# stephane-caron/pink

Hardware: AMD Instinct MI355X
Metric: ik_qp_solves_per_s (higher is better)
Workload: dtype f64

## Files before the change

__graft_entry__.py:

```python

from __future__ import annotations

import hashlib
import os
import subprocess
import sys

ROOT = os.path.dirname(os.path.abspath(__file__))
CSRC = os.path.join(ROOT, "pink_amd", "csrc")
LIB = os.path.join(CSRC, "libpinkhip.so")
HIP_DEPS = ["Makefile", "pinkhip.hip", "tu_kernel.hip", "object_list.h", "ik_sweep.h", "ik_sweepx.h", "ik_stack_rows.h", "ik_rollout.h", "ik_common.h", "ik_kernels_packed.h", "ik_stack_mfma.h",
            "ik_frame_task.h", "ik_kinematics.h", "model_tables.h", "wave.h", "fast_sincos.h", "host_tables.h", "host_plan.h", "dispatch.h",
            "launchers.h", os.path.join(ROOT, "include", "pinkhip.h")]
STAMP = os.path.join(CSRC, "libpinkhip.srchash")


def _source_hash(deps) -> str:
    h = hashlib.sha256()
    for d in deps:
        p = d if os.path.isabs(d) else os.path.join(CSRC, d)
        h.update(os.path.basename(p).encode() + b"\0")
        with open(p, "rb") as f:
            h.update(f.read())
    return h.hexdigest()


def _fresh(target: str, stamp: str, want: str) -> bool:
    return os.path.exists(target) and os.path.exists(stamp) and open(stamp).read().strip() == want


class _BuildLock:

    def __init__(self, name: str):
        self.path = os.path.join(CSRC, name)

    def __enter__(self):
        import fcntl

        self.f = open(self.path, "w")
        fcntl.flock(self.f, fcntl.LOCK_EX)
        return self

    def __exit__(self, *exc):
        import fcntl

        fcntl.flock(self.f, fcntl.LOCK_UN)
        self.f.close()


def build_hip(force: bool = False) -> str:
    want = _source_hash(HIP_DEPS)
    if force or not _fresh(LIB, STAMP, want):
        with _BuildLock(".build.lock"):
            if force or not _fresh(LIB, STAMP, want):
                jobs = str(max(1, len(os.sched_getaffinity(0))))
                subprocess.check_call(["make", "-j", jobs], cwd=CSRC)
                with open(STAMP, "w") as f:
                    f.write(want + "\n")
    return LIB


EMU_PARTS = 16


def build_emulator(force: bool = False) -> str:
    from concurrent.futures import ThreadPoolExecutor

    emu_dir = os.path.join(ROOT, "emu")
    out_dir = os.path.join(ROOT, "tests", "emu")
    target = os.path.join(out_dir, "libpinkemu.so")
    harness = sorted(f for f in os.listdir(emu_dir) if f.startswith("emu_") and f.endswith(".cpp") and not f.endswith("_part.cpp"))
    deps = [os.path.join(emu_dir, f) for f in harness + ["emu_part.cpp", "emu_lanes.h", "emu_registry.h", "wave_emu.h"]] + [WAVE_PROBE_KERNEL, MASK_PROBE_KERNEL] + \
           [os.path.join(CSRC, f) for f in ("ik_common.h", "dispatch.h", "wave.h", "fast_sincos.h", "ik_kernels_packed.h", "ik_sweep.h", "ik_sweepx.h", "ik_stack_rows.h",
                                            "ik_rollout.h", "ik_stack_mfma.h", "ik_frame_task.h", "ik_kinematics.h", "model_tables.h", "host_tables.h", "host_plan.h")]
    stamp, want = os.path.join(out_dir, "libpinkemu.srchash"), _source_hash(deps)
    if force or not _fresh(target, stamp, want):
        with _BuildLock(".build_emu.lock"):
            if force or not _fresh(target, stamp, want):
                objdir = os.path.join(emu_dir, "build")
                os.makedirs(objdir, exist_ok=True)
                os.makedirs(out_dir, exist_ok=True)
                cxx = ["g++", "-O1", "-std=c++17", "-fPIC", "-Wno-psabi"]
                jobs = [cxx + ["-c", os.path.join(emu_dir, f), "-o", os.path.join(objdir, f[:-4] + ".o")] for f in harness]
                for k in range(EMU_PARTS):
                    jobs.append(cxx + [f"-DEMU_PART={k}", f"-DEMU_NPARTS={EMU_PARTS}", "-c", os.path.join(emu_dir, "emu_part.cpp"),
                                       "-o", os.path.join(objdir, f"emu_part_{k}.o")])
                workers = max(1, min(len(jobs), len(os.sched_getaffinity(0))))
                with ThreadPoolExecutor(workers) as pool:
                    list(pool.map(subprocess.check_call, jobs))
                objs = [j[-1] for j in jobs]
                subprocess.check_call(["g++", "-shared", "-o", target + ".tmp"] + objs)
                os.replace(target + ".tmp", target)
                with open(stamp, "w") as f:
                    f.write(want + "\n")
    return target


WAVE_PROBE_DIR = os.path.join(ROOT, "tests", "wave")
WAVE_PROBE_KERNEL = os.path.join(WAVE_PROBE_DIR, "wave_probe_kernel.h")
WAVE_PROBE_LIB = os.path.join(WAVE_PROBE_DIR, "libwaveprobe.so")
MASK_PROBE_KERNEL = os.path.join(WAVE_PROBE_DIR, "lane_mask_probe_kernel.h")
MASK_PROBE_LIB = os.path.join(WAVE_PROBE_DIR, "liblanemaskprobe.so")


def _build_probe(source: str, kernel: str, lib: str, force: bool) -> str:
    deps = [os.path.join(WAVE_PROBE_DIR, source), kernel, os.path.join(CSRC, "wave.h"), os.path.join(CSRC, "fast_sincos.h")]
    stamp, want = lib[:-3] + ".srchash", _source_hash(deps)
    if force or not _fresh(lib, stamp, want):
        with _BuildLock(".build_probe.lock"):
            if force or not _fresh(lib, stamp, want):
                import shutil

                hipcc = os.environ.get("HIPCC") or shutil.which("hipcc") or "/opt/rocm/bin/hipcc"
                subprocess.check_call([hipcc, "--offload-arch=gfx950", "-O3", "-std=c++17", "-fPIC", "-shared", deps[0], "-o", lib + ".tmp"])
                os.replace(lib + ".tmp", lib)
                with open(stamp, "w") as f:
                    f.write(want + "\n")
    return lib


def build_wave_probe(force: bool = False) -> str:
    return _build_probe("wave_probe.hip", WAVE_PROBE_KERNEL, WAVE_PROBE_LIB, force)


def build_lane_mask_probe(force: bool = False) -> str:
    return _build_probe("lane_mask_probe.hip", MASK_PROBE_KERNEL, MASK_PROBE_LIB, force)


def build() -> None:
    build_hip()
    build_wave_probe()
    build_lane_mask_probe()
    sys.path.insert(0, ROOT)
    from oracle import c_oracle

    c_oracle.build()
    build_emulator()
    import pink_amd
    from pink_amd import _lib

    lib = _lib.load_library()
    for name in _lib.ABI_SYMBOLS:
        getattr(lib, name)


def smoke() -> None:
    sys.path.insert(0, ROOT)
    import numpy as np

    from oracle import c_oracle
    from pink_amd import synthetic
    from pink_amd.batch_solver import BatchSolver

    build_hip()
    solver = BatchSolver(device_id=0)
    try:
        for name, B in (("ur5", 64), ("draco3", 256), ("jvrc", 64)):
            terms = synthetic.make_terms(name, B, bounds="tight")
            ref = c_oracle.solve_ik_batch(**synthetic.pink_form(terms))
            out = solver.solve(synthetic.pack(terms))
            assert (out.status == 0).all() and (ref["status"] == 0).all()
            err = float(np.abs(out.dq - ref["dq"]).max())
            print(f"smoke {name}: B={B} max|dq - dq_ref| = {err:.3e}")
            assert err < 1e-8, err
    finally:
        solver.close()


if __name__ == "__main__":
    build()
    if len(sys.argv) > 1 and sys.argv[1] == "smoke":
        smoke()
```

pink_amd/csrc/ik_common.h:

```cpp
#pragma once

#include <cmath>
#include <cstdint>
#include <type_traits>

#ifndef PINKHIP_GROUP_LARGE
#define PINKHIP_GROUP_LARGE 8
#endif
#ifndef PINKHIP_GROUP_SMALL
#define PINKHIP_GROUP_SMALL 4
#endif

#if defined(PINKHIP_TRACE) && !defined(__HIP_DEVICE_COMPILE__)
#include <cstdio>
#define PINKHIP_TRACEF(cond, ...)        \
  do {                                   \
    if (cond) std::printf(__VA_ARGS__);  \
  } while (0)
#else
#define PINKHIP_TRACEF(cond, ...)
#endif

namespace pinkhip {

template <int NV>
constexpr int group_size() {
  return NV >= 24 ? PINKHIP_GROUP_LARGE : PINKHIP_GROUP_SMALL;
}

template <int I, int N, class F>
__device__ __forceinline__ void static_for(F &&f) {
  if constexpr (I < N) {
    f(std::integral_constant<int, I>{});
    static_for<I + 1, N>(f);
  }
}
template <int W, int J>
__device__ __forceinline__ double add_in_lane(double t, double d) {
  static_assert((W == 16 || W == 32 || W == 64) && J >= 0 && J < W, "lane of a group of whole rows of 16 lanes");
#if defined(__HIP_DEVICE_COMPILE__)
  constexpr unsigned long long one = 1ull << J;
  constexpr unsigned long long m = W == 64 ? one : W == 32 ? one | (one << 32) : one | (one << 16) | (one << 32) | (one << 48);
  unsigned slo, shi;
  asm("s_mov_b32 %1, exec_lo\n\ts_mov_b32 %2, exec_hi\n\t"
      "s_and_b32 exec_lo, %1, %4\n\ts_and_b32 exec_hi, %2, %5\n\t"
      "v_add_f64 %0, %0, %3\n\t"
      "s_mov_b32 exec_lo, %1\n\ts_mov_b32 exec_hi, %2"
      : "+v"(t), "=&s"(slo), "=&s"(shi)
      : "v"(d), "n"(static_cast<int>(m & 0xFFFFFFFFull)), "n"(static_cast<int>(m >> 32))
      : "scc");
  return t;
#else
  return ((lane_id() & (W - 1)) == J) ? t + d : t;
#endif
}

template <int W, int N, int BIT, class F>
__device__ __forceinline__ double transpose_reduce(F v) {
  const int lane = lane_id();
  if constexpr ((1 << BIT) >= W) {
    static_assert(N == 1, "N <= W values fold to one per lane");
    return v(std::integral_constant<int, 0>{});
  } else {
    constexpr int H = (N + 1) / 2;
    double nx[H];
    const bool up = ((lane >> BIT) & 1) != 0;
    static_for<0, H>([&](auto M) {
      constexpr int m = decltype(M)::value;
      const double a = v(std::integral_constant<int, 2 * m>{});
      double b = 0.0;
      if constexpr (2 * m + 1 < N) b = v(std::integral_constant<int, 2 * m + 1>{});
      nx[m] = (up ? b : a) + lane_shfl(up ? a : b, lane ^ (1 << BIT));
    });
    return transpose_reduce<W, H, BIT + 1>([&](auto K) { return nx[decltype(K)::value]; });
  }
}

typedef double TabVec16 __attribute__((vector_size(128)));
typedef double TabVec8 __attribute__((vector_size(64)));
template <bool HALF>
struct TabVecSel {
  typedef TabVec16 type;
};
template <>
struct TabVecSel<true> {
  typedef TabVec8 type;
};
template <int NT>
struct TabRegs {
  static constexpr int NVEC = (NT + 15) / 16;
  static_assert(NVEC >= 1 && NVEC <= 4, "at most 64 tableau columns");
  static constexpr bool kHalfLast = NT - 16 * (NVEC - 1) <= 8;
  template <int K>
  using Vec = typename TabVecSel<(K == NVEC - 1) && kHalfLast>::type;
  Vec<0> v0;
  Vec<1> v1;
  Vec<2> v2;
  Vec<3> v3;
  template <int K>
  __device__ __forceinline__ Vec<K> tuple() const {
    if constexpr (K == 0) return v0;
    else if constexpr (K == 1) return v1;
    else if constexpr (K == 2) return v2;
    else return v3;
  }
  template <int J>
  __device__ __forceinline__ double get() const {
    static_assert(J >= 0 && J < NT, "tableau column");
    const Vec<J / 16> t = tuple<J / 16>();
    return t[J % 16];
  }
  template <int J>
  __device__ __forceinline__ void set(double x) {
    static_assert(J >= 0 && J < NT, "tableau column");
    Vec<J / 16> t = tuple<J / 16>();
    t[J % 16] = x;
    if constexpr (J / 16 == 0) v0 = t;
    else if constexpr (J / 16 == 1) v1 = t;
    else if constexpr (J / 16 == 2) v2 = t;
    else v3 = t;
  }
  __device__ __forceinline__ void clear() {
    v0 = Vec<0>{};
    v1 = Vec<1>{};
    v2 = Vec<2>{};
    v3 = Vec<3>{};
  }
  __device__ __forceinline__ double at_uniform(int p) const {
    const int hi = p >> 4;
    const int lo = opaque_uniform(p & 15);
    const int lo8 = kHalfLast ? opaque_uniform(p & 7) : lo;
    const Vec<0> t0 = v0;
    double r = t0[NVEC == 1 ? lo8 : lo];
    if constexpr (NVEC > 1) {
      const Vec<1> t1 = v1;
      const double r1 = t1[NVEC == 2 ? lo8 : lo];
      r = (hi == 1) ? r1 : r;
    }
    if constexpr (NVEC > 2) {
      const Vec<2> t2 = v2;
      const double r2 = t2[NVEC == 3 ? lo8 : lo];
      r = (hi == 2) ? r2 : r;
    }
    if constexpr (NVEC > 3) {
      const Vec<3> t3 = v3;
      const double r3 = t3[lo8];
      r = (hi == 3) ? r3 : r;
    }
    return r;
  }
  template <int W>
  __device__ __forceinline__ double at_group_uniform(int p) const {
    constexpr int G = kWave / W;
    static_assert(G == 1 || G == 2, "one or two reads per wave");
    const int p0 = bcast_i(p, 0);
    double c = at_uniform(p0 < 0 ? 0 : p0);
    if constexpr (G == 2) {
      const int p1 = bcast_i(p, W);
      const double c1 = at_uniform(p1 < 0 ? 0 : p1);
      c = (lane_id() >= W) ? c1 : c;
    }
    return (p >= 0) ? c : 0.0;
  }
};

struct alignas(16) Pair {
  double a, b;
};

constexpr int STATUS_OPTIMAL = 0;
constexpr int STATUS_MAX_ITER = 1;
constexpr int STATUS_INFEASIBLE = 2;
constexpr int STATUS_NOT_PD = 3;
constexpr int STATUS_BREAKDOWN = 4;
constexpr int STATUS_ROUTED = 5;
constexpr int PATH_TABLEAU = 0, PATH_HANDOVER = 1, PATH_ROUTED = 2, PATH_GI = 3;
constexpr int kPathShift = 24;

struct KernelArgs {
  long long B;
  int nv, Kd, K, md;
  int n_eq;
  int n_dtasks;
  int n_barriers;
  int cost_batched;
  int max_iter;
  int lds_pitch;
  int rank_deficient;
  int n_free_lead;
  double damping, dt;
  double out_scale;
  const double *J, *e, *cost, *lb, *ub, *Gd, *hd, *c_extra;
  const double *row_gain;
  const double *row_lm;
  const int *dtask_col0;
  const int *dtask_row0;
  const int *dtask_k;
  const int *barrier_rows;
  const double *barrier_safe_gain;
  double *dq;
  int *status;
  int *iters;
  double *H_out, *c_out;
  const uint8_t *active_in;
  uint8_t *active_out;
};


}
```

pink_amd/csrc/ik_sweep.h:

```cpp
#pragma once

#include "ik_common.h"
#include "ik_kernels_packed.h"
#include "ik_stack_rows.h"

#ifdef PINKHIP_SECTION_CLOCK
#ifndef PINKHIP_TICK
static __device__ unsigned long long pinkhip_clock[16];
#define PINKHIP_TICK(k)                                                        \
  do {                                                                         \
    if (clock_on) {                                                            \
      const unsigned long long now_ = __builtin_readcyclecounter();            \
      if (lane == 0) atomicAdd(&pinkhip_clock[k], now_ - clock_prev);          \
      clock_prev = __builtin_readcyclecounter();                               \
    }                                                                          \
  } while (0)
#endif
#else
#ifndef PINKHIP_TICK
#define PINKHIP_TICK(k)
#endif
#endif

#ifndef PINKHIP_SWEEP_COLUMN_CHAINS
#define PINKHIP_SWEEP_COLUMN_CHAINS(NT) 2
#endif

#ifndef PINKHIP_SWEEP_CERT_TOL
#define PINKHIP_SWEEP_CERT_TOL 1e-12
#endif
#ifndef PINKHIP_STACK_DEPTH
#define PINKHIP_STACK_DEPTH 1
#endif
#ifndef PINKHIP_STACK_DEPTH_WIDE
#define PINKHIP_STACK_DEPTH_WIDE 2
#endif
#ifndef PINKHIP_SWEEP_INDEXED_COLUMN
#define PINKHIP_SWEEP_INDEXED_COLUMN 1
#endif
#ifndef PINKHIP_SWEEP_ROUTE_COND
#define PINKHIP_SWEEP_ROUTE_COND 1e8
#endif
#ifndef PINKHIP_SWEEP_PPM
#define PINKHIP_SWEEP_PPM 1
#endif
#ifndef PINKHIP_SWEEP_PPM_CRASH
#define PINKHIP_SWEEP_PPM_CRASH 1
#endif
#ifndef PINKHIP_ROLLOUT_PPM_DENSE
#define PINKHIP_ROLLOUT_PPM_DENSE 0
#endif
#ifndef PINKHIP_ROLLOUT_PPM_VIRTUAL
#define PINKHIP_ROLLOUT_PPM_VIRTUAL 0
#endif
#ifndef PINKHIP_SWEEP_PPM_DENSE
#define PINKHIP_SWEEP_PPM_DENSE 1
#endif
#ifdef PINKHIP_SWEEP_DEBUG_WHY
#define PINKHIP_WHY(k) why = (k) + 10 * status_before
#else
#define PINKHIP_WHY(k)
#endif
#ifndef PINKHIP_SWEEP_PPM_MIN_CURV
#define PINKHIP_SWEEP_PPM_MIN_CURV 1e-5
#endif
#ifndef PINKHIP_SWEEP_PPM_MURTY_AFTER
#define PINKHIP_SWEEP_PPM_MURTY_AFTER(nv) (4 * (nv) + 20)
#endif

#ifndef PINKHIP_SWEEP_DIAG_REGISTER
#define PINKHIP_SWEEP_DIAG_REGISTER(Src) (!Src::kOnTheFly)
#endif
#ifndef PINKHIP_SWEEP_LATE_ADDRESSES
#define PINKHIP_SWEEP_LATE_ADDRESSES(Src) (!Src::kOnTheFly)
#endif
#ifndef PINKHIP_SWEEP_LANE_MASKS
#define PINKHIP_SWEEP_LANE_MASKS(Src) (!Src::kOnTheFly)
#endif

namespace pinkhip {

template <int NV, int MD, int W>
struct SweepLds {
  static __host__ __device__ constexpr int tri(int i) { return i * (i + 1) / 2; }
  static constexpr int oC = (NV * (NV + 1) / 2 + 1) & ~1;
  static constexpr int GP = W + 2;
  static constexpr int oG = oC + W;
  static constexpr int oR = oG + MD * GP;
  static constexpr int stride = oR + W;
};

template <int NVT, int MD, int W, class Src = HbmTerms, bool WARM = false>
__device__ __forceinline__ int ik_sweep_instance(const KernelArgs &a, long long block, Src *terms = nullptr) {
  constexpr int NE = NVT > W ? NVT - W : 0;
  constexpr int NV = NVT - NE;
  static_assert(NE == 0 || (NE <= 2 && MD == 0 && !Src::kOnTheFly), "front coordinates are eliminated in the box-only stack + solve kernel");
  constexpr int NT = NV + MD;
  static_assert((W == 16 || W == 32 || W == 64) && NT <= W && NV % 2 == 0 && MD >= 0, "group of whole rows of 16 lanes");
  constexpr bool DENSE = MD > 0;
  constexpr bool DREG = PINKHIP_SWEEP_DIAG_REGISTER(Src);
  constexpr bool LM = PINKHIP_SWEEP_LANE_MASKS(Src);
  constexpr bool PPM = !DENSE && PINKHIP_SWEEP_PPM;
  constexpr bool PPMD = DENSE && PINKHIP_SWEEP_PPM && PINKHIP_SWEEP_PPM_DENSE && (!Src::kOnTheFly || PINKHIP_ROLLOUT_PPM_DENSE);
  constexpr bool PPX = PPM || PPMD;
  constexpr bool LMP = LM && PPM;
  static_assert(!WARM || PPM, "a warm start is a start of the principal pivoting of the box-only instantiations");
  constexpr int G = kWave / W;
  constexpr double INF = INFINITY;
  constexpr double BIG = 1e300;
  using BcT = Bcast<W>;

  const int lane = lane_id();
  const int g = lane / W, li = lane & (W - 1);
  const int nvs = a.nv;
  const int nv = nvs - NE;
  const int md = DENSE ? a.md : 0, n_eq = DENSE ? a.n_eq : 0;
#ifdef PINKHIP_SECTION_CLOCK
  const bool clock_on = (block & 63) == 0;
  unsigned long long clock_prev = __builtin_readcyclecounter();
#endif
  long long b = block * G + g;
  const bool valid = b < a.B;
  if (!valid) b = a.B - 1;
  WaveSplit ws;
  ws.first = (block * G < a.B - 1) ? block * G : a.B - 1;
  ws.rel = static_cast<unsigned>(b - ws.first);
  const unsigned vo = ws.rel * static_cast<unsigned>(nvs) + li;

  const bool in = li < nv;
  const int dr = li - NV;
  const bool dlane = DENSE && dr >= 0 && dr < md;

  double T[NT];
#pragma unroll
  for (int j = 0; j < NT; ++j) T[j] = 0.0;
  double ci = 0.0, mu_l = 0.0, dadd = 0.0;
  double ci_d = 0.0, mu_d = 0.0, lbv = -INF, ubv = INF, hv = 0.0, ginv = 1.0;
  double front_dadd[NE > 0 ? NE : 1] = {}, front_c[NE > 0 ? NE : 1] = {};
  bool front_free = true;
  auto others = [&]() {
    if (in) {
      if constexpr (!Src::kOnTheFly) {
        lbv = (a.lb + (ws.first * (long long)nvs + NE))[vo];
        ubv = (a.ub + (ws.first * (long long)nvs + NE))[vo];
      }
      if constexpr (PINKHIP_WAVE_SPLIT(Src)) dadd = stack_diag_tasks<Src>(a, ws, terms, NE + li, ci_d, mu_d);
      else dadd = stack_diag_tasks<Src>(a, b, terms, NE + li, ci_d, mu_d);
      if constexpr (PINKHIP_WAVE_SPLIT(Src)) {
        if (a.c_extra) ci_d += (a.c_extra + (ws.first * (long long)nvs + NE))[vo];
      } else {
        if (a.c_extra) ci_d += a.c_extra[b * (long long)nvs + NE + li];
      }
    }
    if constexpr (NE > 0) {
#pragma unroll
      for (int x = 0; x < NE; ++x) {
        double mu_x = 0.0;
        front_dadd[x] = stack_diag_tasks<Src>(a, b, terms, x, front_c[x], mu_x);
        if (a.c_extra) front_c[x] += a.c_extra[b * (long long)nvs + x];
        if (li == x) mu_d += mu_x;
        front_free = front_free && a.lb[b * (long long)nvs + x] == -INF && a.ub[b * (long long)nvs + x] == INF;
      }
    }
    if constexpr (DENSE && !Src::kOnTheFly) {
      if (md > 0) {
        const double *Gb = a.Gd + b * (long long)md * nv;
        static_for<0, MD>([&](auto Dc) {
          constexpr int d = decltype(Dc)::value;
          T[NV + d] = (in && d < md) ? Gb[(long long)d * nv + li] : 0.0;
        });
        if (dlane) hv = a.hd[b * (long long)md + dr];
      }
    }
  };
  StackFront<NE> front;
  double hii = 0.0;
  if constexpr (NE > 0) {
    KernelArgs af = a;
    af.J = a.J + NE;
    stack_rows_bcast<NV, W, 8, Src, PINKHIP_STACK_DEPTH, NE, DREG>(af, b, terms, in, li, T, ci, mu_l, others, &front, &hii, ws);
  } else {
    stack_rows_bcast<NV, W, 8, Src, (NT > 34 ? PINKHIP_STACK_DEPTH_WIDE : PINKHIP_STACK_DEPTH), 0, DREG>(a, b, terms, in, li, T, ci, mu_l, others, nullptr, &hii, ws);
  }
  ci += ci_d;
  mu_l += mu_d;
  double diag = a.damping + group_sum<W>(mu_l);

  if constexpr (DENSE) {
    if (md > 0) {
      const double *Gb = Src::kOnTheFly ? nullptr : a.Gd + b * (long long)md * nv;
      if constexpr (Src::kOnTheFly) {
        static_for<0, MD>([&](auto Dc) {
          constexpr int d = decltype(Dc)::value;
          T[NV + d] = (in && d < md) ? terms->dense_col(d) : 0.0;
        });
      }
      if constexpr (Src::kOnTheFly) {
        static_for<0, MD>([&](auto Dc) {
          constexpr int d = decltype(Dc)::value;
          if (d < md) {
            const BcT gb = bcast_prepare<W>(T[NV + d]);
            static_for<0, NV>([&](auto Jc) {
              constexpr int j = decltype(Jc)::value;
              const double v = value_bcast<W, j>(gb);
              if (dr == d) T[j] = v;
            });
          }
        });
      }
      if (dlane) {
        double n2 = 0.0;
        if constexpr (!Src::kOnTheFly) {
          const double *gr = Gb + (long long)dr * nv;
#pragma unroll
          for (int j = 0; j < NV; ++j) T[j] = (j < nv) ? gr[j] : 0.0;
        } else {
          hv = terms->dense_h(dr);
        }
#pragma unroll
        for (int j = 0; j < NV; ++j) n2 += T[j] * T[j];
        ginv = (n2 > 0.0) ? 1.0 / sqrt(n2) : 1.0;
      }
      for (int t = 0; t < a.n_barriers; ++t) {
        const double r = a.barrier_safe_gain[t];
        if (r > 1e-6) {
          const int r0 = a.barrier_rows[t], r1 = a.barrier_rows[t + 1];
          double s = 0.0;
          static_for<0, MD>([&](auto Dc) {
            constexpr int d = decltype(Dc)::value;
            if (in && d >= r0 && d < r1) s += T[NV + d] * T[NV + d];
          });
          s = group_sum<W>(s);
          diag += r / (s * a.dt * a.dt);
        }
      }
    }
  }
  const double diag_u = diag;
  diag += dadd;
  if constexpr (DREG) {
    const double dd = in ? diag : 1.0;
    static_for<0, NV>([&](auto Jc) {
      constexpr int j = decltype(Jc)::value;
      T[j] = add_in_lane<W, j>(T[j], dd);
    });
    hii += dd;
  } else {
    hii = 1.0;
#pragma unroll
    for (int j = 0; j < NV; ++j)
      if (j == li) {
        T[j] += in ? diag : 1.0;
        hii = T[j];
      }
  }
  using SL = SweepLds<NV, MD, W>;
  double *sm = shared_base() + (long long)g * (a.lds_pitch ? a.lds_pitch : SL::stride);
  bool front_bad = false;
  if constexpr (NE > 0) {
    double h00 = group_sum<W>(front.hxx[0]) + diag_u + front_dadd[0];
    double c0 = group_sum<W>(front.cx[0]) + front_c[0];
    double h01 = 0.0, h11 = 1.0, c1 = 0.0;
    if constexpr (NE == 2) {
      h01 = group_sum<W>(front.hxx[1]);
      h11 = group_sum<W>(front.hxx[2]) + diag_u + front_dadd[1];
      c1 = group_sum<W>(front.cx[1]) + front_c[1];
    }
    const double m0 = in ? front.m[0] : 0.0;
    double m1 = (NE == 2 && in) ? front.m[NE - 1] : 0.0;
    front_bad = !(h00 > 0.0);
    const double r0 = fast_rcp(h00);
    {
      const BcT hb = bcast_prepare<W>(m0);
      const double f = -m0 * r0;
      static_for<0, NV>([&](auto Jc) {
        constexpr int j = decltype(Jc)::value;
        T[j] = fma_bcast<W, j>(T[j], hb, f);
      });
      ci = fma(f, c0, ci);
      hii = fma(f, m0, hii);
      if constexpr (NE == 2) {
        m1 = fma(f, h01, m1);
        h11 = fma(-h01 * r0, h01, h11);
        c1 = fma(-h01 * r0, c0, c1);
      }
    }
    double r1 = 0.0;
    if constexpr (NE == 2) {
      front_bad = front_bad || !(h11 > 0.0);
      r1 = fast_rcp(h11);
      const BcT hb = bcast_prepare<W>(m1);
      const double f = -m1 * r1;
      static_for<0, NV>([&](auto Jc) {
        constexpr int j = decltype(Jc)::value;
        T[j] = fma_bcast<W, j>(T[j], hb, f);
      });
      ci = fma(f, c1, ci);
      hii = fma(f, m1, hii);
    }
    wave_sync();
    sm[SL::stride + li] = m0;
    sm[SL::stride + W + li] = m1;
    if (li == 0) {
      double *fs = sm + SL::stride + 2 * W;
      fs[0] = c0, fs[1] = r0, fs[2] = h01, fs[3] = c1, fs[4] = r1;
    }
  }
  wave_sync();
  if (li < NV) {
#pragma unroll
    for (int j = 0; j < NV; ++j)
      if (j <= li) sm[SL::tri(li) + j] = T[j];
  }
  sm[SL::oC + li] = ci;
  if constexpr (DENSE) {
    static_for<0, MD>([&](auto Dc) {
      constexpr int d = decltype(Dc)::value;
      sm[SL::oG + d * SL::GP + li] = (li < NV) ? T[NV + d] : 0.0;
    });
  }
  PINKHIP_TICK(0);

  int status = STATUS_OPTIMAL;
  int why = 0, status_before = 0;
  if constexpr (NE > 0) {
    if (!front_free) status = STATUS_ROUTED;
    else if (front_bad) status = STATUS_NOT_PD;
  }
  double pmin = INF;
  int state = 0;
  if constexpr (Src::kOnTheFly) {
    lbv = in ? terms->lb : -INF;
    ubv = in ? terms->ub : INF;
  }
  constexpr bool GUESS = (PPX && PINKHIP_SWEEP_PPM_CRASH && !Src::kOnTheFly) || WARM;
  double tdiag = (li < NV) ? hii : 0.0;
  if constexpr (GUESS) {
    if (group_first_lane<W>(in && !(hii > 0.0)) < W) status = STATUS_NOT_PD;
    if constexpr (WARM) {
      const uint8_t *hint = a.active_in;
      if (hint) {
        if (in) {
          const int v = hint[b * (long long)nvs + NE + li];
          state = (v == 1 && lbv > -INF) ? 1 : ((v == 2 && ubv < INF) ? 2 : 0);
        }
      } else if constexpr (!Src::kOnTheFly) {
        const double xd = -ci * approx_rcp(hii);
        if (in) state = (xd < lbv) ? 1 : ((xd > ubv) ? 2 : 0);
      }
    } else {
      const double xd = -ci * approx_rcp(hii);
      if (in) state = (xd < lbv) ? 1 : ((xd > ubv) ? 2 : 0);
    }
    const unsigned long long fm = wave_ballot(li < NV && state == 0 && in);
    using FreeMask = typename std::conditional<W == 64, unsigned long long, unsigned>::type;
    FreeMask gfree = static_cast<FreeMask>(fm);
    if constexpr (W == 32) gfree = (lane >= 32) ? static_cast<unsigned>(fm >> 32) : static_cast<unsigned>(fm);
    else if constexpr (W == 16) gfree = static_cast<unsigned>(fm >> (lane & 48)) & 0xFFFFu;
    static_for<0, NV>([&](auto Kc) {
      constexpr int k = decltype(Kc)::value;
      {
        const bool want = ((gfree >> k) & 1) != 0;
        if (lanes_on(want)) {
          BcT xb = bcast_prepare<W>(T[k]);
          const double p = value_bcast<W, k>(xb);
          pmin = min_raw(pmin, want ? p : INF);
          const double rp = fast_rcp(p);
          double own = T[k];
          if constexpr (DREG) opaque(own);
          const double t = T[k] * rp;
          double nt = (li == k) ? rp - 1.0 : -t;
          if (!want) nt = 0.0;
          double tk = (li == k) ? -rp : t;
#if defined(__HIP_DEVICE_COMPILE__)
          asm volatile("" : "+v"(nt), "+v"(xb.r[0]), "+v"(tk));
#endif
          double td = 0.0;
          if constexpr (DREG) td = fma(own, nt, tdiag);
          static_for<0, NT>([&](auto Jc) {
            constexpr int j = decltype(Jc)::value;
            if constexpr (j != k) T[j] = fma_bcast<W, j>(T[j], xb, nt);
          });
          if (want) T[k] = tk;
          if constexpr (DREG) tdiag = (li == k) ? T[k] : td;
        }
      }
    });
  }
  if constexpr (!GUESS) {
    static_for<0, NV>([&](auto Kc) {
      constexpr int k = decltype(Kc)::value;
      if (k < nv) {
        const BcT xb = bcast_prepare<W>(T[k]);
        const double p = value_bcast<W, k>(xb);
        pmin = min_raw(pmin, p);
        const double rp = fast_rcp(p);
        const double t = T[k] * rp;
        const double nt = (li == k) ? rp - 1.0 : -t;
        static_for<0, NT>([&](auto Jc) {
          constexpr int j = decltype(Jc)::value;
          if constexpr (j != k) T[j] = fma_bcast<W, j>(T[j], xb, nt);
        });
        if constexpr (DREG) tdiag = (li == k) ? -rp : fma(T[k], nt, tdiag);
        T[k] = (li == k) ? -rp : t;
      }
    });
  }
  if (!(pmin > 0.0)) status = STATUS_NOT_PD;
  PINKHIP_TICK(1);
  if constexpr (DREG) {
    if (li >= NT) tdiag = 0.0;
  } else {
    tdiag = 0.0;
#pragma unroll
    for (int j = 0; j < NT; ++j)
      if (j == li) tdiag = T[j];
  }

  double x = 0.0, u = 0.0;
  {
    double vstart = in ? ci : 0.0;
    if constexpr (PPX) {
      if (state != 0) vstart = -((state == 1) ? lbv : ubv);
    }
    const BcT cb = bcast_prepare<W>(vstart);
    double r0 = 0.0, r1 = 0.0;
    static_for<0, NV>([&](auto Jc) {
      constexpr int j = decltype(Jc)::value;
      if constexpr (j % 2 == 0) r0 = fma_bcast<W, j>(r0, cb, T[j]);
      else r1 = fma_bcast<W, j>(r1, cb, T[j]);
    });
    x = in ? r0 + r1 : 0.0;
    if (dlane) u = hv + (r0 + r1);
    if constexpr (PPX) {
      if (state != 0) x -= ci;
    }
    if constexpr (PPMD) {
      if (dlane) x = u;
    }
  }
  double zd0 = -tdiag;
  if constexpr (PPMD) {
    const double hmax = -group_min<W>(in ? -hii : 0.0);
    zd0 = (li < NV) ? approx_rcp(hii) : approx_rcp(ginv * ginv * hmax);
  }
  {
    const double hii0 = (li < NV && in) ? sm[SL::tri(li < NV ? li : 0) + (li < NV ? li : 0)] : 0.0;
    const double kest = -group_min<W>((PPX && state != 0) ? -hii0 * approx_rcp(tdiag) : hii0 * tdiag);
    PINKHIP_TRACEF(li == 0, "[sweep g%d] kest %.3e\n", g, kest);
    if (status == STATUS_OPTIMAL && !(kest <= PINKHIP_SWEEP_ROUTE_COND)) status = STATUS_ROUTED;
  }
  PINKHIP_TICK(2);

  const KernelArgs *late = &a;
  if constexpr (!Src::kOnTheFly) late = kernarg_reload<KernelArgs>(a);
  const double tol = 1e-13 * (nv > 8 ? nv * 0.125 : 1.0);
  const double thr_lo = -tol * (1.0 + fabs(lbv)), thr_up = -tol * (1.0 + fabs(ubv));
  const double thr_d = -tol * (1.0 + fabs(hv) * ginv);
  const int max_iter = late->max_iter > 0 ? late->max_iter : 20 * (nv + md) + 50;
  const bool empty_box_somewhere = wave_any(in && ubv - lbv < (thr_lo > thr_up ? thr_lo : thr_up));
  double phi = 0.0, xfree = 1.0;
  int it = 0, eq_next = 0, src = 0, kind = 0;
  double uplus = 0.0;
  double blo = lbv, bhi = ubv, tlo = thr_lo, thi = thr_up;
  double thr_row = 0.0;
  if constexpr (PPMD) {
    thr_row = thr_d * fast_rcp(ginv);
    if (li >= NV) {
      blo = dlane ? 0.0 : -INF;
      bhi = INF;
      tlo = (dlane && dr >= n_eq) ? thr_row : -INF;
      thi = 0.0;
    }
  }
  if constexpr (PPX) {
    if (state != 0) {
      blo = (state == 1) ? -INF : 0.0;
      bhi = (state == 1) ? 0.0 : INF;
      tlo = 0.0;
      thi = 0.0;
    }
    if (empty_box_somewhere) {
      const bool empty = group_first_lane<W>(in && ubv - lbv < (thr_lo > thr_up ? thr_lo : thr_up)) < W;
      if (empty && status == STATUS_OPTIMAL) status = STATUS_INFEASIBLE;
    }
  }
  bool at_point = false;
  bool running = (status == STATUS_OPTIMAL);
  bool need_sel = true;
  bool refined = (status == STATUS_ROUTED);
  unsigned long long run_m = 0, ref_m = 0, atp_m = 0;
  if constexpr (LMP) {
    run_m = wave_ballot(status == STATUS_OPTIMAL);
    ref_m = wave_ballot(status == STATUS_ROUTED);
  }
  int nref = 0;
  double dprev = 0.0;

  auto krow_times = [&](double v) -> double {
    const BcT vb = bcast_prepare<W>(v);
    constexpr bool LATE = PINKHIP_SWEEP_LATE_ADDRESSES(Src);
    int lo_ = li;
#if defined(__HIP_DEVICE_COMPILE__)
    if constexpr (LATE) asm volatile("" : "+v"(lo_));
#endif
    const int base = (lo_ < NV) ? SL::tri(lo_) : SL::oG + (dlane ? dr : 0) * SL::GP;
    const double *const rowp = sm + base, *const colp = sm + lo_;
    double h0 = 0.0, h1 = 0.0;
    static_for<0, NV>([&](auto Jc) {
      constexpr int j = decltype(Jc)::value;
      double hv_;
      if constexpr (LATE) {
        const double *const pj = (j > lo_) ? colp : rowp + (j - SL::tri(j));
        hv_ = pj[SL::tri(j)];
      } else {
        hv_ = sm[(li < NV && j > li) ? SL::tri(j) + li : base + j];
      }
      if constexpr (j % 2 == 0) h0 = fma_bcast<W, j>(h0, vb, hv_);
      else h1 = fma_bcast<W, j>(h1, vb, hv_);
    });
    return h0 + h1;
  };
  auto residual = [&](bool &fails) -> double {
    const double kx = krow_times(in ? x : 0.0);
    const double ci_ = in ? sm[SL::oC + li] : 0.0;
    double grad = in ? kx + ci_ : 0.0;
    bool arow = false;
    if constexpr (DENSE) {
      if (md > 0) {
        arow = dlane && state == 1;
        const BcT lamb = bcast_prepare<W>(arow ? u : 0.0);
        double gl = 0.0;
        static_for<0, MD>([&](auto Dc) {
          constexpr int d = decltype(Dc)::value;
          gl = fma_bcast<W, NV + d>(gl, lamb, sm[SL::oG + d * SL::GP + li]);
        });
        if (in) grad += gl;
      }
    }
    const double hii = in ? sm[SL::tri(li < NV ? li : 0) + (li < NV ? li : 0)] : 0.0;
    const double gsc = group_min<W>(-hii) * group_min<W>(in ? -fabs(x) : 0.0) - group_min<W>(-fabs(ci_));
    const double gtol = PINKHIP_SWEEP_CERT_TOL * gsc;
    fails = false;
    if (in) {
      if (state == 0) fails = !(fabs(grad) <= gtol && x - lbv >= 10.0 * thr_lo && ubv - x >= 10.0 * thr_up);
      else fails = (state == 1) ? !(grad >= -gtol) : !(grad <= gtol);
    }
#if defined(PINKHIP_SWEEP_DEBUG_WHY) && defined(__HIP_DEVICE_COMPILE__)
    if (fails) printf("[cert blk %lld g%d li%d it%d nref%d] state %d x %.17g lb %.17g ub %.17g grad %.3e gtol %.3e thr %.3e %.3e\n", block, g, li, it, nref, state, x,
                      lbv, ubv, grad, gtol, thr_lo, thr_up);
#endif
    double r = (in && state == 0) ? grad : 0.0;
    if constexpr (DENSE) {
      if (dlane) {
        const double slack = (hv - kx) * ginv;
        if (arow) {
          r = kx - hv;
          fails = !(fabs(slack) <= -10.0 * thr_d) || (dr >= n_eq && !(u >= -gtol * ginv));
        } else if (state == 0 && dr >= n_eq) {
          fails = !(slack >= 10.0 * thr_d);
        }
      }
    }
    return r;
  };

#ifndef PINKHIP_SWEEP_LDS_COLUMN
#define PINKHIP_SWEEP_LDS_COLUMN 0
#endif
  double sdiag_run = tdiag;
  double *rowbuf = sm + SL::oR;
  constexpr bool IDX = PINKHIP_SWEEP_INDEXED_COLUMN && !PINKHIP_SWEEP_LDS_COLUMN && W >= 32;
  TabRegs<IDX ? NT : 1> R;
  R.clear();
  if constexpr (IDX) {
    static_for<0, NT>([&](auto Jc) {
      constexpr int j = decltype(Jc)::value;
      R.template set<j>(T[j]);
    });
  }
  auto tget = [&](auto Jc) -> double {
    constexpr int j = decltype(Jc)::value;
    if constexpr (IDX) return R.template get<j>();
    else return T[j];
  };
  auto tset = [&](auto Jc, double v) {
    constexpr int j = decltype(Jc)::value;
    if constexpr (IDX) R.template set<j>(v);
    else T[j] = v;
  };
  auto column_of = [&](int p) -> double {
    if constexpr (IDX) {
      return R.template at_group_uniform<W>(p);
    } else if constexpr (PINKHIP_SWEEP_LDS_COLUMN) {
      if (li == p) {
        Pair *dst = reinterpret_cast<Pair *>(__builtin_assume_aligned(rowbuf, 16));
#pragma unroll
        for (int j = 0; j + 1 < NT; j += 2) dst[j >> 1] = Pair{T[j], T[j + 1]};
        if constexpr (NT % 2) rowbuf[NT - 1] = T[NT - 1];
      }
      wave_sync();
      const double c = rowbuf[li < NT ? li : 0];
      wave_sync();
      return (p >= 0 && li < NT) ? c : 0.0;
    } else {
      const BcT eb = bcast_indicator<W>(p);
      constexpr int NC = PINKHIP_SWEEP_COLUMN_CHAINS(NT);
      double c[NC] = {};
      static_for<0, NT>([&](auto Jc) {
        constexpr int j = decltype(Jc)::value;
        c[j % NC] = fma_bcast<W, j>(c[j % NC], eb, tget(Jc));
      });
      if constexpr (NC == 4) return (c[0] + c[1]) + (c[2] + c[3]);
      else return c[0] + c[1];
    }
  };

  auto pivot_on = [&](int pi, double col, double pvt, double rp, double sg) {
    double t = col * rp;
    double cp = col;
    if (li == pi) {
      t = 1.0 - sg * rp;
      cp = pvt - sg;
    }
    const BcT xb = bcast_prepare<W>(cp);
    const double nt = -t;
    static_for<0, NT>([&](auto Jc) {
      constexpr int j = decltype(Jc)::value;
      tset(Jc, fma_bcast<W, j>(tget(Jc), xb, nt));
    });
    sdiag_run = fma(cp, nt, sdiag_run);
    tdiag = (li == pi) ? -rp : tdiag - t * col;
  };

  bool ppm_mode = PPX;
  bool restoring = false;
  const bool cand_lane = in || (DENSE && dlane && dr >= n_eq);
  const bool eq_lane = DENSE && dlane && dr < n_eq;
  int trips = 0;
  int rare_after = (PINKHIP_SWEEP_PPM_MURTY_AFTER(nv + md) < max_iter) ? PINKHIP_SWEEP_PPM_MURTY_AFTER(nv + md) : max_iter;
  if constexpr (LMP) rare_after = wave_uniform(rare_after);

  for (;;) {
    if constexpr (LMP) {
      ++trips;
      running = lane_pred(run_m), refined = lane_pred(ref_m), at_point = lane_pred(atp_m);
    }
    double viol = 0.0;
    int nb_src = 0;
    bool iseq = false;
    if constexpr (PPX) {
      bool some_sel;
      if constexpr (LMP) some_sel = run_m != 0;
      else some_sel = wave_any(running && ppm_mode);
      if (some_sel) {
        const bool sel = running && ppm_mode;
        const double slo = x - blo, sup = bhi - x;
        bool ok_lane = in, nonbasic = state != 0;
        if constexpr (DENSE) {
          nonbasic = (li < NV) ? (state != 0) : (state == 0);
          ok_lane = cand_lane && (!restoring || ((li < NV) ? (state != 0) : (state == 1)));
        }
        const bool vlo = ok_lane && slo < tlo, vup = ok_lane && sup < thi;
        viol = vlo ? slo : sup;
        if constexpr (DENSE) {
          if (eq_lane) viol = slo;
        }
        const float zf = fabsf(static_cast<float>(tdiag));
        const float wz = (zf > 1e-30f) ? approx_rcpf(zf) : 1e30f;
        const float fv = static_cast<float>(viol);
        float key = -(fv * fv) * wz;
        if constexpr (LMP) {
          if (trips > rare_after) {
#if defined(__HIP_DEVICE_COMPILE__)
            asm volatile("" : "+v"(key));
#endif
            if (it > PINKHIP_SWEEP_PPM_MURTY_AFTER(nv + md)) key = static_cast<float>(li - 64);
          }
        } else {
          if (it > PINKHIP_SWEEP_PPM_MURTY_AFTER(nv + md)) key = static_cast<float>(li - 64);
        }
        float best32;
        if constexpr (LMP) best32 = group_min32<W>((vlo || vup) ? key32_packf_quiet(key, li | (vlo ? 0 : 64) | (nonbasic ? 128 : 0)) : 3.0e38f);
        else best32 = group_min32<W>((vlo || vup) ? key32_packf(key, li | (vlo ? 0 : 64) | (nonbasic ? 128 : 0)) : 3.0e38f);
        bool conv = false;
        if (sel) {
          if (DENSE && !restoring && eq_next < n_eq) {
            src = NV + eq_next;
            kind = 0;
            nb_src = 1;
            iseq = true;
          } else if (!(best32 < 0.0f)) {
            if (DENSE && restoring) {
              ppm_mode = false;
              need_sel = true;
            } else {
              running = false;
            }
            conv = DENSE;
          } else {
            const int pl = key32_payload(best32);
            src = pl & 63;
            kind = (pl >> 6) & 1;
            nb_src = pl >> 7;
          }
        }
        if constexpr (LMP) run_m &= ~wave_ballot(!(best32 < 0.0f));
        if constexpr (DENSE) {
          if (conv) {
            u = (li < NV) ? ((state == 1) ? -x : ((state == 2) ? x : 0.0)) : x;
            phi = (li < NV) ? ((state == 1) ? -1.0 : ((state == 2) ? 1.0 : 0.0)) : ((dlane && state == 1 && dr >= n_eq) ? 1.0 : 0.0);
            xfree = ((li < NV) ? (state != 0) : (state == 1)) ? 0.0 : 1.0;
            if (li < NV && state != 0) x = (state == 1) ? lbv : ubv;
          }
        }
      }
    }
    if (!PPM && wave_any(running && !ppm_mode && need_sel)) {
      const bool sel = running && !ppm_mode && need_sel;
      const double slo = x - lbv, sup = ubv - x;
      const bool vlo = in && slo < thr_lo, vup = in && sup < thr_up;
      const float zf = static_cast<float>(-tdiag);
      const float wz = (zf > 1e-30f) ? approx_rcpf(zf) : 1e30f;
      const float flo = static_cast<float>(slo), fup = static_cast<float>(sup);
      const bool clo = vlo && state == 0;
      bool has = clo;
      float key = -(flo * flo) * wz;
      int id = li;
      if (vup && state == 0) {
        const float ku = -(fup * fup) * wz;
        if (!clo || ku < key) key = ku, id = 64 + li;
        has = true;
      }
      if constexpr (DENSE) {
        if (dlane && dr >= n_eq && state == 0 && u * ginv < thr_d) {
          const float fu = static_cast<float>(u);
          key = -(fu * fu) * wz;
          has = true;
        }
      }
      const float best32 = group_min32<W>(has ? key32_packf(key, id) : 3.0e38f);
      const bool none = !(best32 < 0.0f);
      bool bad = false;
      if (empty_box_somewhere) bad = group_first_lane<W>((vlo && vup) || (state != 0 && in && (vlo || vup))) < W;
      if (sel) {
        uplus = 0.0;
        if (bad) {
          status = STATUS_INFEASIBLE;
          running = false;
        } else if (DENSE && eq_next < n_eq) {
          src = NV + eq_next;
          kind = 3;
          need_sel = false;
        } else if (none) {
          running = false;
        } else {
          const int pl = key32_payload(best32);
          src = pl & 63;
          if constexpr (DENSE) kind = (src >= NV) ? 2 : (pl >> 6) & 1;
          else kind = (pl >> 6) & 1;
          need_sel = false;
        }
      }
    }
    if constexpr (LMP) {
      if (running) ++it;
      if (trips > rare_after) {
#if defined(__HIP_DEVICE_COMPILE__)
        asm volatile("" : "+v"(it));
#endif
        const bool over = it > max_iter;
        if (running && over) status = STATUS_MAX_ITER;
        running = running && !over;
        run_m &= ~wave_ballot(over);
      }
    } else if (running) {
      if (++it > max_iter) {
        status = STATUS_MAX_ITER;
        running = false;
      }
      if constexpr (PPMD) {
        if (ppm_mode && it > 2 * PINKHIP_SWEEP_PPM_MURTY_AFTER(nv + md)) restoring = true;
      }
    }
    bool closing;
    if constexpr (LMP) closing = run_m == 0;
    else closing = !wave_any(running);
    const bool ref = closing && !refined;
    if constexpr (LMP) {
      if (closing && ~ref_m == 0) break;
    } else {
      if (closing && !wave_any(ref)) break;
    }
    const bool act = running;
    PINKHIP_TICK(3);

    double col;
    if (!(PINKHIP_SWEEP_LDS_COLUMN || IDX) || closing) {
      BcT eb = bcast_indicator<W>(act ? src : -1);
      double rres = 0.0, sdiag = 0.0;
      bool cert_fails = false, illc = false;
      if (closing) {
        if constexpr (PPM) {
          if (!at_point) {
            if (state != 0) x = (state == 1) ? lbv : ubv;
            at_point = true;
          }
          if constexpr (LMP) atp_m = ~0ull;
        }
        rres = residual(cert_fails);
        if constexpr (PPX) {
          const double hii_ = (in && state == 0) ? sm[SL::tri(li < NV ? li : 0) + (li < NV ? li : 0)] : 0.0;
          const double kfin = -group_min<W>(hii_ * tdiag);
          illc = !(kfin <= PINKHIP_SWEEP_ROUTE_COND);
        }
        cert_fails = group_first_lane<W>(cert_fails) < W;
        if (!ref || status != STATUS_OPTIMAL) rres = 0.0;
        sdiag = sdiag_run;
        eb = bcast_select<W>(ref, bcast_prepare<W>(rres), eb);
      }
      constexpr int NC = PINKHIP_SWEEP_COLUMN_CHAINS(NT);
      double c[NC] = {};
      static_for<0, NT>([&](auto Jc) {
        constexpr int j = decltype(Jc)::value;
        c[j % NC] = fma_bcast<W, j>(c[j % NC], eb, tget(Jc));
      });
      if constexpr (NC == 4) col = (c[0] + c[1]) + (c[2] + c[3]);
      else col = c[0] + c[1];
      if (closing) {
        const bool arow_ = DENSE && dlane && state == 1;
        const double dbv = (ref && ((in && state == 0) || arow_)) ? col + (tdiag - sdiag) * rres : 0.0;
        const double dxv = in ? dbv : 0.0;
        const double xmax = -group_min<W>(in ? -fabs(x) : 0.0);
        const bool more = group_first_lane<W>(fabs(dxv) > 1e-9 * fabs(x) + 1e-11 * (1.0 + xmax)) < W;
        const double dmax = -group_min<W>(-fabs(dxv));
        const bool sane = dmax <= ((nref == 0) ? 0.1 * xmax : 0.5 * dprev);
        if (ref) {
          if (status != STATUS_OPTIMAL || illc) {
            status_before = status;
            status = STATUS_BREAKDOWN;
            PINKHIP_WHY(2);
            refined = true;
          } else if (!cert_fails && !more) {
            if (sane) x += dxv;
            refined = true;
          } else if (sane && nref < 3) {
            x += dxv;
            if (arow_) u += dbv;
            dprev = dmax;
            ++nref;
          } else {
            status = STATUS_BREAKDOWN;
            PINKHIP_WHY(3);
#if defined(PINKHIP_SWEEP_DEBUG_WHY) && defined(__HIP_DEVICE_COMPILE__)
            if (li == 0) printf("[close blk %lld g%d it%d nref%d] cert_fails %d more %d sane %d dmax %.3e xmax %.3e dprev %.3e\n", block, g, it, nref, (int)cert_fails,
                                (int)more, (int)sane, dmax, xmax, dprev);
#endif
            refined = true;
          }
        }
        if constexpr (LMP) {
          ref_m = wave_ballot(refined);
          if (~ref_m == 0) break;
        } else {
          if (!wave_any(!refined)) break;
        }
      }
    } else {
      col = column_of(act ? src : -1);
    }
    if (li == src) col = tdiag;
    int pi = -1;
    double pvt = 1.0, rp = 0.0;
    double sg = -1.0;
    if constexpr (PPX) {
      if (PPM || wave_any(act && ppm_mode)) {
        const bool actP = act && ppm_mode;
        const double vs = group_bcast<W>(viol, src);
        const double num = kind ? vs : -vs;
        const double pv = group_bcast<W>(tdiag, src);
        PINKHIP_TICK(4);
        const double rpv = fast_rcp(pv);
        const double sgp = nb_src ? 1.0 : -1.0;
        bool act2 = actP;
        if constexpr (!DENSE) {
          if constexpr (LMP) {
            const unsigned long long bad_m = wave_ballot(!(pv * sgp > 0.0)) & run_m;
            if (bad_m != 0) {
#if defined(__HIP_DEVICE_COMPILE__)
              asm volatile("" : "+v"(status));
#endif
              if (lane_pred(bad_m)) status = STATUS_NOT_PD;
            }
            run_m &= ~bad_m;
            running = lane_pred(run_m);
            act2 = running;
          } else if (actP && !(pv * sgp > 0.0)) {
            status = STATUS_NOT_PD;
            running = false;
            act2 = false;
          }
        } else {
          const double zr = group_bcast<W>(zd0, src);
          const bool recip = (src < NV) == (nb_src != 0);
          const bool irregular = actP && !((recip ? pv : -pv) > (recip ? 0.0 : PINKHIP_SWEEP_PPM_MIN_CURV * zr));
          double hs = 0.0;
          if (wave_any(irregular && iseq)) hs = group_bcast<W>(hv, src);
          if (irregular) {
            act2 = false;
            PINKHIP_TRACEF(li == 0, "[ppm g%d it%d] irregular: src %d kind %d nonbasic %d pv %.3e zref %.3e num %.3e eq %d restoring %d\n", g, it, src,
                           kind, nb_src, pv, zr, num, (int)iseq, (int)restoring);
            if (iseq && fabs(num) <= 1e-9 * (1.0 + fabs(hs))) {
              ++eq_next;
            } else if (!restoring) {
              restoring = true;
            } else {
              status = STATUS_BREAKDOWN;
              PINKHIP_WHY(1);
              running = false;
            }
          }
        }
        const double nu = act2 ? -num * rpv : 0.0;
        x = fma(-col, nu, x);
        if (act2) {
          pi = src;
          pvt = pv;
          rp = rpv;
          sg = sgp;
          if (li == src) {
            if (!DENSE || li < NV) {
              if (state != 0) {
                x = ((state == 1) ? lbv : ubv) + nu;
                state = 0;
                blo = lbv;
                bhi = ubv;
                tlo = thr_lo;
                thi = thr_up;
              } else {
                x = -nu;
                state = kind + 1;
                blo = kind ? 0.0 : -INF;
                bhi = kind ? INF : 0.0;
                tlo = 0.0;
                thi = 0.0;
// ... 257 lines not shown
```

Baseline: 187.3 million.

## Split box-only PPM sweep into dedicated pivot loop and separate refinement loop

For box-only lane-masked instantiations, the unified sweep loop is replaced with a specialised pivoting loop that carries only the principal-pivoting path, followed by a separate refinement loop. This drops per-trip mode checks and branches for restoring and Murty fallback from the hot loop, aiming to shorten the instruction stream per pivot. An emulator variant with an early Murty threshold is also built to exercise the rare path. It duplicates a lot of logic, so the two paths could diverge in behaviour, and the refinement loop still carries a dummy pivot per iteration.

```diff
diff --git a/__graft_entry__.py b/__graft_entry__.py
--- a/__graft_entry__.py
+++ b/__graft_entry__.py
@@ -61,26 +61,29 @@
 
 
 EMU_PARTS = 16
+EMU_VARIANTS = {"murty": ["-DPINKHIP_SWEEP_PPM_MURTY_AFTER(nv)=2"]}
 
 
-def build_emulator(force: bool = False) -> str:
+def build_emulator(force: bool = False, variant: str = "") -> str:
     from concurrent.futures import ThreadPoolExecutor
 
     emu_dir = os.path.join(ROOT, "emu")
     out_dir = os.path.join(ROOT, "tests", "emu")
-    target = os.path.join(out_dir, "libpinkemu.so")
+    suffix = "_" + variant if variant else ""
+    extra = EMU_VARIANTS[variant] if variant else []
+    target = os.path.join(out_dir, f"libpinkemu{suffix}.so")
     harness = sorted(f for f in os.listdir(emu_dir) if f.startswith("emu_") and f.endswith(".cpp") and not f.endswith("_part.cpp"))
     deps = [os.path.join(emu_dir, f) for f in harness + ["emu_part.cpp", "emu_lanes.h", "emu_registry.h", "wave_emu.h"]] + [WAVE_PROBE_KERNEL, MASK_PROBE_KERNEL] + \
            [os.path.join(CSRC, f) for f in ("ik_common.h", "dispatch.h", "wave.h", "fast_sincos.h", "ik_kernels_packed.h", "ik_sweep.h", "ik_sweepx.h", "ik_stack_rows.h",
                                             "ik_rollout.h", "ik_stack_mfma.h", "ik_frame_task.h", "ik_kinematics.h", "model_tables.h", "host_tables.h", "host_plan.h")]
-    stamp, want = os.path.join(out_dir, "libpinkemu.srchash"), _source_hash(deps)
+    stamp, want = os.path.join(out_dir, f"libpinkemu{suffix}.srchash"), _source_hash(deps)
     if force or not _fresh(target, stamp, want):
         with _BuildLock(".build_emu.lock"):
             if force or not _fresh(target, stamp, want):
-                objdir = os.path.join(emu_dir, "build")
+                objdir = os.path.join(emu_dir, "build" + suffix)
                 os.makedirs(objdir, exist_ok=True)
                 os.makedirs(out_dir, exist_ok=True)
-                cxx = ["g++", "-O1", "-std=c++17", "-fPIC", "-Wno-psabi"]
+                cxx = ["g++", "-O1", "-std=c++17", "-fPIC", "-Wno-psabi"] + extra
                 jobs = [cxx + ["-c", os.path.join(emu_dir, f), "-o", os.path.join(objdir, f[:-4] + ".o")] for f in harness]
                 for k in range(EMU_PARTS):
                     jobs.append(cxx + [f"-DEMU_PART={k}", f"-DEMU_NPARTS={EMU_PARTS}", "-c", os.path.join(emu_dir, "emu_part.cpp"),
@@ -136,6 +139,8 @@
 
     c_oracle.build()
     build_emulator()
+    for variant in EMU_VARIANTS:
+        build_emulator(variant=variant)
     import pink_amd
     from pink_amd import _lib
 
diff --git a/pink_amd/csrc/ik_common.h b/pink_amd/csrc/ik_common.h
--- a/pink_amd/csrc/ik_common.h
+++ b/pink_amd/csrc/ik_common.h
@@ -161,6 +161,17 @@
       c = (lane_id() >= W) ? c1 : c;
     }
     return (p >= 0) ? c : 0.0;
+  }
+  template <int W>
+  __device__ __forceinline__ double at_group_uniform_on(int p, bool on) const {
+    constexpr int G = kWave / W;
+    static_assert(G == 1 || G == 2, "one or two reads per wave");
+    double c = at_uniform(bcast_i(p, 0));
+    if constexpr (G == 2) {
+      const double c1 = at_uniform(bcast_i(p, W));
+      c = (lane_id() >= W) ? c1 : c;
+    }
+    return on ? c : 0.0;
   }
 };
 
diff --git a/pink_amd/csrc/ik_sweep.h b/pink_amd/csrc/ik_sweep.h
--- a/pink_amd/csrc/ik_sweep.h
+++ b/pink_amd/csrc/ik_sweep.h
@@ -76,6 +76,9 @@
 #endif
 #ifndef PINKHIP_SWEEP_LANE_MASKS
 #define PINKHIP_SWEEP_LANE_MASKS(Src) (!Src::kOnTheFly)
+#endif
+#ifndef PINKHIP_SWEEP_SPLIT_CLOSING
+#define PINKHIP_SWEEP_SPLIT_CLOSING(Src) (!Src::kOnTheFly)
 #endif
 
 namespace pinkhip {
@@ -104,6 +107,7 @@
   constexpr bool PPMD = DENSE && PINKHIP_SWEEP_PPM && PINKHIP_SWEEP_PPM_DENSE && (!Src::kOnTheFly || PINKHIP_ROLLOUT_PPM_DENSE);
   constexpr bool PPX = PPM || PPMD;
   constexpr bool LMP = LM && PPM;
+  constexpr bool SPLIT = LMP && PINKHIP_SWEEP_SPLIT_CLOSING(Src);
   static_assert(!WARM || PPM, "a warm start is a start of the principal pivoting of the box-only instantiations");
   constexpr int G = kWave / W;
   constexpr double INF = INFINITY;
@@ -641,6 +645,154 @@
   int rare_after = (PINKHIP_SWEEP_PPM_MURTY_AFTER(nv + md) < max_iter) ? PINKHIP_SWEEP_PPM_MURTY_AFTER(nv + md) : max_iter;
   if constexpr (LMP) rare_after = wave_uniform(rare_after);
 
+  if constexpr (SPLIT) {
+    auto pivot_lane = [&](bool me, double col, double pvt, double rp, double sg) {
+      double t = col * rp;
+      double cp = col;
+      if (me) {
+        t = 1.0 - sg * rp;
+        cp = pvt - sg;
+      }
+      const BcT xb = bcast_prepare<W>(cp);
+      const double nt = -t;
+      static_for<0, NT>([&](auto Jc) {
+        constexpr int j = decltype(Jc)::value;
+        tset(Jc, fma_bcast<W, j>(tget(Jc), xb, nt));
+      });
+      sdiag_run = fma(cp, nt, sdiag_run);
+      tdiag = me ? -rp : tdiag - t * col;
+    };
+    while (run_m != 0) {
+      ++trips;
+      const double slo = x - blo, sup = bhi - x;
+      const bool vlo = in && slo < tlo, vup = in && sup < thi;
+      const double viol = vlo ? slo : sup;
+      const float zf = fabsf(static_cast<float>(tdiag));
+      const float wz = (zf > 1e-30f) ? approx_rcpf(zf) : 1e30f;
+      const float fv = static_cast<float>(viol);
+      float key = -(fv * fv) * wz;
+      if (trips > rare_after) {
+#if defined(__HIP_DEVICE_COMPILE__)
+        asm volatile("" : "+v"(key));
+#endif
+        if (it > PINKHIP_SWEEP_PPM_MURTY_AFTER(nv + md)) key = static_cast<float>(li - 64);
+      }
+      const float best32 = group_min32<W>((vlo || vup) ? key32_packf_quiet(key, li | (vlo ? 0 : 64) | ((state != 0) ? 128 : 0)) : 3.0e38f);
+      run_m &= ~wave_ballot(!(best32 < 0.0f));
+      running = lane_pred(run_m);
+      const int pl = key32_payload(best32);
+      if (running) src = pl & 63;
+      kind = (pl >> 6) & 1;
+      const int nb_src = pl >> 7;
+      if (running) ++it;
+      if (trips > rare_after) {
+#if defined(__HIP_DEVICE_COMPILE__)
+        asm volatile("" : "+v"(it));
+#endif
+        const bool over = it > max_iter;
+        if (running && over) status = STATUS_MAX_ITER;
+        run_m &= ~wave_ballot(over);
+        running = lane_pred(run_m);
+      }
+      if (run_m == 0) break;
+      PINKHIP_TICK(3);
+      double col;
+      if constexpr (IDX) col = R.template at_group_uniform_on<W>(src, running);
+      else col = column_of(running ? src : -1);
+      if (li == src) col = tdiag;
+      const double vs = group_bcast<W>(viol, src);
+      const double num = kind ? vs : -vs;
+      const double pv = group_bcast<W>(tdiag, src);
+      PINKHIP_TICK(4);
+      const double rpv = fast_rcp(pv);
+      const double sgp = nb_src ? 1.0 : -1.0;
+      const unsigned long long bad_m = wave_ballot(!(pv * sgp > 0.0)) & run_m;
+      if (bad_m != 0) {
+#if defined(__HIP_DEVICE_COMPILE__)
+        asm volatile("" : "+v"(status));
+#endif
+        if (lane_pred(bad_m)) status = STATUS_NOT_PD;
+        run_m &= ~bad_m;
+      }
+      const bool act2 = lane_pred(run_m);
+      const double nu = act2 ? -num * rpv : 0.0;
+      x = fma(-col, nu, x);
+      const bool me = act2 && li == src;
+      if (me) {
+        if (state != 0) {
+          x = ((state == 1) ? lbv : ubv) + nu;
+          state = 0;
+          blo = lbv, bhi = ubv, tlo = thr_lo, thi = thr_up;
+        } else {
+          x = -nu;
+          state = kind + 1;
+          blo = kind ? 0.0 : -INF;
+          bhi = kind ? INF : 0.0;
+          tlo = 0.0, thi = 0.0;
+        }
+      }
+      PINKHIP_TICK(5);
+      PINKHIP_TICK(6);
+      pivot_lane(me, col, pv, act2 ? rpv : 0.0, sgp);
+      PINKHIP_TICK(7);
+    }
+    PINKHIP_TICK(3);
+    if (~ref_m != 0) {
+      refined = lane_pred(ref_m);
+      if (state != 0) x = (state == 1) ? lbv : ubv;
+      for (;;) {
+        const bool ref = !refined;
+        bool cert_fails = false;
+        double rres = residual(cert_fails);
+        const double hii_ = (in && state == 0) ? sm[SL::tri(li < NV ? li : 0) + (li < NV ? li : 0)] : 0.0;
+        const double kfin = -group_min<W>(hii_ * tdiag);
+        const bool illc = !(kfin <= PINKHIP_SWEEP_ROUTE_COND);
+        cert_fails = group_first_lane<W>(cert_fails) < W;
+        if (!ref || status != STATUS_OPTIMAL) rres = 0.0;
+        const double sdiag = sdiag_run;
+        const BcT eb = bcast_select<W>(ref, bcast_prepare<W>(rres), bcast_indicator<W>(-1));
+        constexpr int NC = PINKHIP_SWEEP_COLUMN_CHAINS(NT);
+        double c[NC] = {};
+        static_for<0, NT>([&](auto Jc) {
+          constexpr int j = decltype(Jc)::value;
+          c[j % NC] = fma_bcast<W, j>(c[j % NC], eb, tget(Jc));
+        });
+        double col;
+        if constexpr (NC == 4) col = (c[0] + c[1]) + (c[2] + c[3]);
+        else col = c[0] + c[1];
+        const double dbv = (ref && in && state == 0) ? col + (tdiag - sdiag) * rres : 0.0;
+        const double dxv = in ? dbv : 0.0;
+        const double xmax = -group_min<W>(in ? -fabs(x) : 0.0);
+        const bool more = group_first_lane<W>(fabs(dxv) > 1e-9 * fabs(x) + 1e-11 * (1.0 + xmax)) < W;
+        const double dmax = -group_min<W>(-fabs(dxv));
+        const bool sane = dmax <= ((nref == 0) ? 0.1 * xmax : 0.5 * dprev);
+        if (ref) {
+          if (status != STATUS_OPTIMAL || illc) {
+            status_before = status;
+            status = STATUS_BREAKDOWN;
+            PINKHIP_WHY(2);
+            refined = true;
+          } else if (!cert_fails && !more) {
+            if (sane) x += dxv;
+            refined = true;
+          } else if (sane && nref < 3) {
+            x += dxv;
+            dprev = dmax;
+            ++nref;
+          } else {
+            status = STATUS_BREAKDOWN;
+            PINKHIP_WHY(3);
+            refined = true;
+          }
+        }
+        ref_m = wave_ballot(refined);
+        if (~ref_m == 0) break;
+        if (li == src) col = tdiag;
+        x = fma(-col, 0.0, x);
+        pivot_lane(false, col, 1.0, 0.0, -1.0);
+      }
+    }
+  } else
   for (;;) {
     if constexpr (LMP) {
       ++trips;
```

New measurement: 196.3 million (median of 6 runs). +4.8%, better.
